# moble/scri

Measured on NVIDIA B200. Metric: mode-timesteps/sec through WaveformModes.transform (ell_max=8), higher is better.
Workload: dtype f64

## Files before the change

### scri_b200/csrc/spline_tile.cu

```cuda
#include <cuda.h>
#include <math_constants.h>
#include <stdlib.h>

#include "common.cuh"

namespace scrib200 {

constexpr int ST_COLS = 16;
constexpr int ST_ROWD = 16;
constexpr int ST_BR = 16;
constexpr int ST_TAB6 = 6;
constexpr int FACTOR_RUNIN = 40;
constexpr int ST_MAXBLK = 24;

__device__ __forceinline__ unsigned st_smem_u32(const void* p) { return (unsigned)__cvta_generic_to_shared(p); }

__device__ __forceinline__ int st_idx(int rrel, int c) { return rrel * ST_ROWD + ((((c >> 1) ^ (rrel & 7)) << 1) | (c & 1)); }

__device__ __forceinline__ void nak_row(const double* __restrict__ t, int N, int r, double& sub, double& diag, double& sup,
                                        double& hm, double& hp) {
    hm = t[r] - t[r - 1];
    hp = t[r + 1] - t[r];
    sub = hm;
    diag = 2.0 * (hm + hp);
// ... 245 lines not shown
        int total = 0;
#pragma unroll
        for (int c = 0; c < ST_COLS / 2; ++c) total += s_nch[c];
        const int per = (total + nwarp - 1) / nwarp;
        el = warp * per;
        erem = (total - el < per) ? total - el : per;
        while (ec < ST_COLS / 2 && el >= s_nch[ec]) el -= s_nch[ec++];
        if (erem > 0 && ec < ST_COLS / 2) {
            const int jn = s_jlo[ec] + (el << 5) + lane;
            if (jn < s_jhi[ec]) u_next = up[jn];
        }
    }
    {
        unsigned ok = 0;
        const unsigned mb = st_smem_u32(&s_mbar);
        while (!ok)
            asm volatile("{ .reg .pred p; mbarrier.try_wait.parity.shared::cta.b64 p, [%1], 0; selp.u32 %0, 1, 0, p; }" : "=r"(ok) : "r"(mb) : "memory");
    }

    const int cc = tid & (ST_COLS - 1);
    const int q = qlo + tid / ST_COLS;
    const bool active = (q <= qhi);
    const int qbase = q * ST_BR;
    const int r0 = (qbase > slo) ? qbase : slo;
    const int r1 = (qbase + ST_BR - 1 < shi) ? qbase + ST_BR - 1 : shi;
    const bool full = active && r0 == qbase && r1 == qbase + ST_BR - 1;
    const int rb = qbase - ybase;
    const int c2 = cc >> 1, c1 = cc & 1;
    const double* yq = sY + rb * ST_ROWD + c1;
    double* mq = sD + rb * ST_ROWD + c1;
    const double* tq = sTab + rb * ST_TAB6;
#define YQ(k_) yq[(k_) * ST_ROWD + ((c2 ^ ((k_) & 7)) << 1)]
#define MQ(k_) mq[(k_) * ST_ROWD + ((c2 ^ ((k_) & 7)) << 1)]
#define TQ2(k_, f_) (*reinterpret_cast<const double2*>(tq + (k_) * ST_TAB6 + (f_)))
    double dreg[ST_BR];
    if (full) {
        double yc = YQ(0);
        double dym = yc - YQ(-1);
        double d = 0.0;
#pragma unroll
        for (int k = 0; k < ST_BR; ++k) {
            const double yn = YQ(k + 1);
            const double dy = yn - yc;
            const double2 pq = TQ2(k, 0);
            d = fma(-tq[k * ST_TAB6 + 4], d, pq.x * dy - pq.y * dym);
            dreg[k] = d;
            yc = yn;
            dym = dy;
        }
        sEdgeD[(q - qlo) * ST_COLS + cc] = d;
    } else if (active) {
        double yc = SY(r0, cc);
        double dym = yc - SY(r0 - 1, cc);
        double d = 0.0;
#pragma unroll
        for (int k = 0; k < ST_BR; ++k) {
            dreg[k] = 0.0;
            if (qbase + k >= r0 && qbase + k <= r1) {
                const double yn = YQ(k + 1);
                const double dy = yn - yc;
                const double2 pq = TQ2(k, 0);
                d = fma(-tq[k * ST_TAB6 + 4], d, pq.x * dy - pq.y * dym);
                dreg[k] = d;
                yc = yn;
                dym = dy;
            }
        }
        sEdgeD[(q - qlo) * ST_COLS + cc] = d;
    }
    __syncthreads();
    if (active) {
        double D = 0.0, w = 1.0;
        for (int p = q - 1; p >= qlo; --p) {
            D = fma(w, sEdgeD[(p - qlo) * ST_COLS + cc], D);
            w *= STAB(p * ST_BR + ST_BR - 1, 2);
            if (fabs(w) < 1e-24) break;
        }
        double m = 0.0;
        if (full) {
#pragma unroll
            for (int k = ST_BR - 1; k >= 0; --k) {
                const double2 pc = TQ2(k, 2);
                m = fma(-pc.y, m, fma(pc.x, D, dreg[k]));
                dreg[k] = m;
            }
        } else {
#pragma unroll
            for (int k = ST_BR - 1; k >= 0; --k)
                if (qbase + k >= r0 && qbase + k <= r1) {
                    const double2 pc = TQ2(k, 2);
                    m = fma(-pc.y, m, fma(pc.x, D, dreg[k]));
                    dreg[k] = m;
                }
        }
        sEdgeM[(q - qlo) * ST_COLS + cc] = m;
    }
    __syncthreads();
    if (active) {
        double E = 0.0, w = 1.0;
        for (int p = q + 1; p <= qhi; ++p) {
            E = fma(w, sEdgeM[(p - qlo) * ST_COLS + cc], E);
            w *= STAB(p * ST_BR, 5);
            if (fabs(w) < 1e-24) break;
        }
        if (full) {
#pragma unroll
            for (int k = 0; k < ST_BR; ++k) MQ(k) = fma(tq[k * ST_TAB6 + 5], E, dreg[k]);
        } else {
#pragma unroll
            for (int k = 0; k < ST_BR; ++k)
                if (qbase + k >= r0 && qbase + k <= r1) MQ(k) = fma(tq[k * ST_TAB6 + 5], E, dreg[k]);
        }
    }
#undef YQ
#undef MQ
#undef TQ2
    __syncthreads();
    if (a == 0 && tid < ST_COLS) {
        const double h0 = STT(1) - STT(0), h1 = STT(2) - STT(1);
        SD(0, tid) = ((h0 + h1) * SD(1, tid) - h0 * SD(2, tid)) / h1;
    }
    if (last_tile && tid >= 32 && tid < 32 + ST_COLS) {
        const int c = tid - 32;
        const double hm = STT(N - 2) - STT(N - 3), hp = STT(N - 1) - STT(N - 2);
        SD(N - 1, c) = ((hm + hp) * SD(N - 2, c) - hp * SD(N - 3, c)) / hm;
    }
    if (a == 0 || last_tile) __syncthreads();

    if (MODE == 0) {
        double2* o2 = reinterpret_cast<double2*>(out);
        const int tmask = (1 << tshift) - 1;
        const int64_t jbase = (int64_t)bz * Nout;
        const int64_t ostride = ((int64_t)32 >> tshift) * ((int64_t)G << tshift);
        while (erem > 0 && ec < ST_COLS / 2) {
            const int c = ec;
            const int nrun = (s_nch[c] - el < erem) ? s_nch[c] - el : erem;
            const int j1 = s_jhi[c];
            const int g = bx * (ST_COLS / 2) + c;
            const double k = s_k[c], al = s_al[c], xa = s_xa[c];
            const float slope = s_slope[c];
            int j = s_jlo[c] + (el << 5) + lane;
            const int64_t jg0 = jbase + j;
            double2* optr = o2 + ((((jg0 >> tshift) * G + g) << tshift) + (jg0 & tmask));
            double u = u_next;
            for (int run = 0; run < nrun; ++run, j += 32, optr += ostride) {
                if (run + 1 < nrun) {
                    u_next = (j + 32 < j1) ? up[j + 32] : 0.0;
                }
                if (j < j1) {
            int i = a + __float2int_rd((float)(u - xa) * slope);
            i = max(a, min(i, b - 1));
            double ti = STT(i), ti1 = STT(i + 1);
            double xi = __dmul_rn(k, __dsub_rn(ti, al));
            double xi1 = __dmul_rn(k, __dsub_rn(ti1, al));
            if (!((xi <= u || i == a) && (u < xi1 || i == b - 1))) {
                int lo_s = a, hi_s = b - 1;
                while (lo_s < hi_s) {
                    const int mid = (lo_s + hi_s + 1) >> 1;
                    if (__dmul_rn(k, __dsub_rn(STT(mid), al)) <= u) lo_s = mid; else hi_s = mid - 1;
                }
                i = lo_s;
                ti = STT(i);
                ti1 = STT(i + 1);
                xi = __dmul_rn(k, __dsub_rn(ti, al));
                xi1 = __dmul_rn(k, __dsub_rn(ti1, al));
            }
            const double ht = ti1 - ti;
            const double hx = xi1 - xi;
            float seed;
            asm("rcp.approx.ftz.f32 %0, %1;" : "=f"(seed) : "f"((float)hx));
            double inv_h = (double)seed;
            double e = fma(-hx, inv_h, 1.0);
            if (fabs(e) < 1e-3) {
                inv_h = fma(inv_h, e, inv_h);
                e = fma(-hx, inv_h, 1.0);
                inv_h = fma(inv_h, e, inv_h);
            } else {
                inv_h = 1.0 / hx;
            }
            const double A = (xi1 - u) * inv_h;
            const double B = (u - xi) * inv_h;
            const double h26 = ht * ht * (1.0 / 6.0);
            const double ca = (A * A * A - A) * h26;
            const double cb = (B * B * B - B) * h26;
            const int ir = i - ybase;
            const int o0 = ir * ST_ROWD + ((c ^ (ir & 7)) << 1), o1 = (ir + 1) * ST_ROWD + ((c ^ ((ir + 1) & 7)) << 1);
            const double2 yi = *reinterpret_cast<const double2*>(sY + o0);
            const double2 yi1 = *reinterpret_cast<const double2*>(sY + o1);
            const double2 Mi = *reinterpret_cast<const double2*>(sD + o0);
            const double2 Mi1 = *reinterpret_cast<const double2*>(sD + o1);
            double2 r;
            r.x = A * yi.x + B * yi1.x + (ca * Mi.x + cb * Mi1.x);
            r.y = A * yi.y + B * yi1.y + (ca * Mi.y + cb * Mi1.y);
                    *optr = r;
                }
                u = u_next;
            }
            erem -= nrun;
            el = 0;
            ++ec;
            if (erem > 0 && ec < ST_COLS / 2) {
                const int jn = s_jlo[ec] + lane;
                u_next = (jn < s_jhi[ec]) ? up[jn] : 0.0;
            }
        }
    } else {
        const int rstep = nthr / ST_COLS;
        const bool colok = col0 + cc < G2;
        out += (size_t)bz * N * G2;
        if (MODE == 4) up += (size_t)bz * N * G2;
        auto value = [&](int i, bool& last_row, double& last_val) -> double {
            const double ht = STT(i + 1) - STT(i);
            const double yi = SY(i, cc), yi1 = SY(i + 1, cc);
            const double Mi = SD(i, cc), Mi1 = SD(i + 1, cc);
            last_row = false;
            if (MODE == 1) {
                const double dl = (yi1 - yi) / ht, h6 = ht * (1.0 / 6.0);
                if (i == N - 2) {
                    last_row = true;
                    last_val = dl + h6 * (Mi + 2.0 * Mi1);
                }
                return dl - h6 * (2.0 * Mi + Mi1);
            } else if (MODE == 2) {
                if (i == N - 2) {
                    last_row = true;
                    last_val = Mi1;
                }
                return Mi;
            } else if (MODE == 3) {
                return 0.5 * ht * (yi + yi1) - (ht * ht * ht) * (1.0 / 24.0) * (Mi + Mi1);
            } else {
                const double c1 = (yi1 - yi) / ht - ht * (1.0 / 6.0) * (2.0 * Mi + Mi1);
                const double h2 = ht * ht;
                const double Jv = h2 * (0.5 * yi + ht * (1.0 / 6.0) * c1 + h2 * ((1.0 / 24.0) * Mi + (1.0 / 120.0) * (Mi1 - Mi)));
                return Jv + (colok ? ht * up[(size_t)i * G2 + col0 + cc] : 0.0);
            }
        };
        if (MODE <= 2) {
            for (int i = a + tid / ST_COLS; i < b; i += rstep) {
                bool lr;
                double lv = 0.0;
                const double v = value(i, lr, lv);
                if (!colok) continue;
                out[(size_t)i * G2 + col0 + cc] = v;
                if (lr) out[(size_t)(N - 1) * G2 + col0 + cc] = lv;
            }
        } else {
            constexpr int VMAX = 16;
            double val[VMAX];
            bool lr;
            double lv;
#pragma unroll
            for (int k = 0; k < VMAX; ++k) {
                const int i = a + tid / ST_COLS + k * rstep;
                val[k] = (i < b) ? value(i, lr, lv) : 0.0;
            }
            __syncthreads();
#pragma unroll
            for (int k = 0; k < VMAX; ++k) {
                const int i = a + tid / ST_COLS + k * rstep;
                if (i < b) SD(i, cc) = val[k];
            }
            __syncthreads();
            const int nr = b - a, slen = (nr + ST_BR - 1) / ST_BR;
            for (int id = tid; id < ST_BR * ST_COLS; id += nthr) {
                const int s = id / ST_COLS, c = id - s * ST_COLS;
                const int r0s = a + s * slen, r1s = (r0s + slen < b) ? r0s + slen : b;
                double run = 0.0;
                for (int r = r0s; r < r1s; ++r) {
                    run += SD(r, c);
                    SD(r, c) = run;
                }
                sEdgeD[s * ST_COLS + c] = run;
            }
            __syncthreads();
            if (tid < ST_COLS) {
                double run = 0.0;
#pragma unroll
                for (int p = 0; p < ST_BR; ++p) {
                    const double v = sEdgeD[p * ST_COLS + tid];
                    sEdgeD[p * ST_COLS + tid] = run;
                    run += v;
                }
            }
            __syncthreads();
            if (colok) {
                const float rs = 1.0f / (float)slen;
                for (int i = a + tid / ST_COLS; i < b; i += rstep) {
                    int s = (int)((float)(i - a) * rs);
                    s -= (s * slen > i - a);
                    s += ((s + 1) * slen <= i - a);
                    out[(size_t)(i + 1) * G2 + col0 + cc] = SD(i, cc) + sEdgeD[s * ST_COLS + cc];
                    if (i == 0) out[col0 + cc] = 0.0;
                }
            }
        }
    }
#undef SY
#undef SD
#undef STAB
#undef STT
}

__global__ void __launch_bounds__(1024)
tile_scan_totals_kernel(double* __restrict__ x, int64_t N, int C, int body, int ntiles) {
    __shared__ double tot[32][33];
    const int col = blockIdx.x * 32 + threadIdx.x, seg = threadIdx.y;
    const int per = (ntiles + 31) / 32;
    const int k0 = seg * per, k1 = (k0 + per < ntiles) ? k0 + per : ntiles;
    const bool ok = col < C;
    auto at = [&](int k) -> double* {
        const int64_t last = (int64_t)(k + 1) * body;
        return x + (last < N - 1 ? last : N - 1) * C + col;
    };
    double run = 0.0;
    if (ok) {
        for (int k = k0; k < k1; k += 8) {
            double v[8];
#pragma unroll
            for (int j = 0; j < 8; ++j) v[j] = (k + j < k1) ? *at(k + j) : 0.0;
#pragma unroll
            for (int j = 0; j < 8; ++j)
                if (k + j < k1) {
                    run += v[j];
                    *at(k + j) = run;
                }
        }
    }
    tot[seg][threadIdx.x] = run;
    __syncthreads();
    if (!ok || seg == 0) return;
    double pre = 0.0;
    for (int p = 0; p < seg; ++p) pre += tot[p][threadIdx.x];
    for (int k = k0; k < k1; k += 8) {
        double v[8];
#pragma unroll
        for (int j = 0; j < 8; ++j) v[j] = (k + j < k1) ? *at(k + j) : 0.0;
#pragma unroll
        for (int j = 0; j < 8; ++j)
            if (k + j < k1) *at(k + j) = v[j] + pre;
    }
}

__global__ void __launch_bounds__(128)
tile_scan_add_kernel(double* __restrict__ x, int64_t N, int C, int body) {
    const int col = blockIdx.x * 128 + threadIdx.x;
    if (col >= C) return;
    const int64_t first = (int64_t)(blockIdx.y + 1) * body;
    if (first >= N - 1) return;
    const int64_t last = first + body < N - 1 ? first + body : N - 1;
    const double base = x[first * C + col];
    double* p = x + (first + 1) * C + col;
    int left = (int)(last - first - 1);
    for (; left >= 8; left -= 8, p += 8 * (size_t)C) {
        double v[8];
#pragma unroll
        for (int j = 0; j < 8; ++j) v[j] = p[(size_t)j * C];
#pragma unroll
        for (int j = 0; j < 8; ++j) p[(size_t)j * C] = v[j] + base;
    }
    for (; left > 0; --left, p += C) *p += base;
}

static int launch_tile_scan(double* x, int64_t N, int C, int body, cudaStream_t st) {
    const unsigned gx = (unsigned)((C + 127) / 128);
    const int64_t ntiles = (N - 1 + body - 1) / body;
    if (ntiles <= 1) return SCRIB200_OK;
    tile_scan_totals_kernel<<<(unsigned)((C + 31) / 32), dim3(32, 32), 0, st>>>(x, N, C, body, (int)ntiles);
    SCRIB200_CHECK_LAUNCH("spline_calculus(scan: totals)");
    tile_scan_add_kernel<<<dim3(gx, (unsigned)(ntiles - 1)), 128, 0, st>>>(x, N, C, body);
    SCRIB200_CHECK_LAUNCH("spline_calculus(scan: add)");
    return SCRIB200_OK;
}

static int tile_box_rows(int body, int halo) {
    const int ymax = body + 2 * halo + 2;
    return (((ymax + 7 + 1) / 2) + 7) & ~7;
}

static size_t tile_smem_bytes(int body, int halo) {
    const size_t nrows = 2 * (size_t)tile_box_rows(body, halo);
    const size_t nblk = std::max<size_t>(((size_t)body + 2 * halo) / ST_BR, ST_BR);
    return (2 * nrows * ST_ROWD + nrows * ST_TAB6 + nrows + 2 * nblk * ST_COLS + 5 * ST_COLS) * sizeof(double) + 1024;
}

static void resolve_tile(int& halo, int& body) {
    if (halo <= 0) halo = 32;
    if (body <= 0) {
        static const int env_body = [] { const char* e = std::getenv("SCRIB200_TILE_BODY"); return e ? std::atoi(e) : 0; }();
        body = env_body > 0 ? env_body : ((halo <= 32) ? 240 : (halo <= 64 ? 176 : 128));
    }
}

typedef CUresult (*TensorMapEncodeTiledFn)(CUtensorMap*, CUtensorMapDataType, cuuint32_t, void*, const cuuint64_t*, const cuuint64_t*,
                                            const cuuint32_t*, const cuuint32_t*, CUtensorMapInterleave, CUtensorMapSwizzle,
                                            CUtensorMapL2promotion, CUtensorMapFloatOOBfill);

static TensorMapEncodeTiledFn tensor_map_encoder() {
    static TensorMapEncodeTiledFn fn = nullptr;
    if (fn == nullptr) {
        void* p = nullptr;
        cudaDriverEntryPointQueryResult qres;
        if (cudaGetDriverEntryPoint("cuTensorMapEncodeTiled", &p, cudaEnableDefault, &qres) == cudaSuccess && qres == cudaDriverEntryPointSuccess)
            fn = reinterpret_cast<TensorMapEncodeTiledFn>(p);
    }
    return fn;
}

template <int MODE>
static int launch_tile(const double* t, int64_t n_times, const double* F, int G, const double* kconf, const double* alpha,
                       const double* tab, const double* uprm, int64_t n_out, double* out, int tshift, int halo, int body,
                       void* workspace, size_t workspace_bytes, void* stream, const char* name, int n_series = 1,
                       int64_t row_lo = 0, int64_t row_hi = -1) {
    SCRIB200_REQUIRE(n_times < (int64_t)2147483000 && n_out < (int64_t)2147483000, "%s: series longer than 2^31 samples", name);
    resolve_tile(halo, body);
    SCRIB200_REQUIRE(halo % ST_BR == 0 && body % ST_BR == 0, "%s: body=%d and halo=%d must be multiples of %d", name, body, halo, ST_BR);
    const size_t smem = tile_smem_bytes(body, halo);
    const int nblk = (body + 2 * halo) / ST_BR;
    const int box_rows = tile_box_rows(body, halo);
    SCRIB200_REQUIRE(nblk <= ST_MAXBLK && smem <= 220 * 1024 && box_rows <= 256, "%s: body=%d halo=%d does not fit one CTA", name, body, halo);
    const int64_t ntiles = (n_times - 1 + body - 1) / body;
    SCRIB200_REQUIRE(ntiles <= 65535, "%s: too many time tiles (%lld); raise `body`", name, (long long)ntiles);
    SCRIB200_REQUIRE(n_series >= 1 && n_series <= 65535 && (int64_t)n_series * n_times < (int64_t)2147483000,
                     "%s: n_series=%d (x %lld rows) out of range", name, n_series, (long long)n_times);
    TensorMapEncodeTiledFn encode = tensor_map_encoder();
    SCRIB200_REQUIRE(encode != nullptr, "%s: cuTensorMapEncodeTiled is not available from this driver", name);
    CUtensorMap tmF;
    {
        const cuuint64_t gdim[2] = {(cuuint64_t)(2 * (int64_t)G), (cuuint64_t)((int64_t)n_series * n_times)};
        const cuuint64_t gstride[1] = {(cuuint64_t)(2 * (int64_t)G) * sizeof(double)};
        const cuuint32_t box[2] = {(cuuint32_t)ST_COLS, (cuuint32_t)box_rows};
        const cuuint32_t estr[2] = {1, 1};
        const CUresult r = encode(&tmF, CU_TENSOR_MAP_DATA_TYPE_FLOAT64, 2, const_cast<double*>(F), gdim, gstride, box, estr,
                                  CU_TENSOR_MAP_INTERLEAVE_NONE, CU_TENSOR_MAP_SWIZZLE_128B, CU_TENSOR_MAP_L2_PROMOTION_L2_128B,
                                  CU_TENSOR_MAP_FLOAT_OOB_FILL_NONE);
        SCRIB200_REQUIRE(r == CUDA_SUCCESS, "%s: cuTensorMapEncodeTiled failed (%d) for a [%lld, %d] grid array", name, (int)r,
                         (long long)n_series * n_times, 2 * G);
    }
    const int threads = ((nblk * ST_COLS + 31) / 32) * 32;
    const bool small = threads <= 320;
    if (small) cudaFuncSetAttribute(spline_tile_kernel<MODE, 320>, cudaFuncAttributeMaxDynamicSharedMemorySize, (int)smem);
    else cudaFuncSetAttribute(spline_tile_kernel<MODE, ST_MAXBLK * ST_COLS>, cudaFuncAttributeMaxDynamicSharedMemorySize, (int)smem);
    int64_t tile_lo = 0, tile_hi = ntiles;
    if (row_hi >= 0) {
        tile_lo = (row_lo > 0 ? row_lo : 0) / body;
        tile_hi = (row_hi + body - 1) / body;
        if (tile_hi > ntiles) tile_hi = ntiles;
        if (tile_lo >= tile_hi) return SCRIB200_OK;
    }
    dim3 grid((2 * G + ST_COLS - 1) / ST_COLS, (unsigned)(tile_hi - tile_lo), (unsigned)n_series);
    int* J = nullptr;
    int* flags = nullptr;
    if (MODE == 0) {
        const size_t need = ((size_t)(ntiles + 1) * G + (size_t)ntiles * grid.x) * sizeof(int);
        SCRIB200_REQUIRE(workspace && workspace_bytes >= need, "%s: workspace too small (%zu < %zu)", name, workspace_bytes, need);
        J = reinterpret_cast<int*>(workspace);
        const int64_t total = (ntiles + 1) * (int64_t)G;
        spline_jrange_kernel<<<(unsigned)((total + 255) / 256), 256, 0, (cudaStream_t)stream>>>(
            t, (int)n_times, G, kconf, alpha, uprm, (int)n_out, body, (int)ntiles, J);
        SCRIB200_CHECK_LAUNCH(name);
        flags = J + total;
        const int64_t nflags = ntiles * (int64_t)grid.x;
        spline_tile_flags_kernel<<<(unsigned)((nflags + 255) / 256), 256, 0, (cudaStream_t)stream>>>(J, (int)ntiles, G, (int)grid.x, flags);
        SCRIB200_CHECK_LAUNCH(name);
    }
    if (small)
        spline_tile_kernel<MODE, 320><<<grid, threads, smem, (cudaStream_t)stream>>>(
            tmF, t, (int)n_times, G, kconf, alpha, tab, uprm, (int)n_out, out, tshift, body, halo, J, flags, box_rows, (int)tile_lo);
    else
        spline_tile_kernel<MODE, ST_MAXBLK * ST_COLS><<<grid, threads, smem, (cudaStream_t)stream>>>(
            tmF, t, (int)n_times, G, kconf, alpha, tab, uprm, (int)n_out, out, tshift, body, halo, J, flags, box_rows, (int)tile_lo);
    SCRIB200_CHECK_LAUNCH(name);
    return SCRIB200_OK;
}

}

extern "C" int scrib200_spline_prepare(const double* t, int64_t n_times, double gamma_factor, int divide, double time_translation,
                                       const double* kconf, const double* alpha, int G, double* tab, double* uprm,
                                       double* info, void* stream) {
    using namespace scrib200;
    SCRIB200_REQUIRE(t && tab && info, "spline_prepare: null pointer");
    SCRIB200_REQUIRE(n_times >= 4 && n_times < (int64_t)2147483000, "spline_prepare: a cubic interpolating spline needs at least 4 knots; got %lld",
                     (long long)n_times);
    SCRIB200_REQUIRE(uprm == nullptr || (kconf && alpha && G > 0), "spline_prepare: output times need kconf, alpha, G");
    SCRIB200_REQUIRE(aligned16(tab), "spline_prepare: tab must be 16-byte aligned");
    cudaStream_t st = (cudaStream_t)stream;
    spline_info_init_kernel<<<1, 32, 0, st>>>(info, (double)n_times);
    const unsigned blocks = (unsigned)((n_times + 255) / 256);
    spline_factor_kernel<<<blocks, 256, 0, st>>>(t, (int)n_times, tab, gamma_factor, divide,
                                                 time_translation, kconf, alpha, G, uprm, info);
    SCRIB200_CHECK_LAUNCH("spline_prepare(factor)");
    spline_decay_kernel<<<blocks, 256, 0, st>>>(tab, (int)n_times, info);
    SCRIB200_CHECK_LAUNCH("spline_prepare(decay)");
    return SCRIB200_OK;
}

extern "C" size_t scrib200_spline_remap_workspace_bytes(int64_t n_times, int G, int halo, int body) {
    using namespace scrib200;
    resolve_tile(halo, body);
    if (n_times < 2 || body <= 0) return 16;
    const int64_t ntiles = (n_times - 1 + body - 1) / body;
    const size_t ncg = (size_t)(2 * G + ST_COLS - 1) / ST_COLS;
    return ((size_t)(ntiles + 1) * (size_t)G + (size_t)ntiles * ncg) * sizeof(int) + 16;
}

extern "C" int scrib200_spline_remap(const double* t, int64_t n_times, const double* F, int G, const double* kconf,
                                     const double* alpha, const double* tab, const double* uprm, int64_t n_out,
                                     double* out, int tile, int halo, int body, int n_series, void* workspace,
                                     size_t workspace_bytes, void* stream) {
    using namespace scrib200;
    SCRIB200_REQUIRE(t && F && kconf && alpha && tab && uprm && out, "spline_remap: null pointer");
    SCRIB200_REQUIRE(n_times >= 4, "spline_remap: a cubic interpolating spline needs at least 4 knots; got %lld",
                     (long long)n_times);
    int tshift = 0;
    while ((1 << tshift) < tile) ++tshift;
    SCRIB200_REQUIRE(G > 0 && (tile == 0 || (tile >= 2 && tile <= 32 && (1 << tshift) == tile)),
                     "spline_remap: G=%d, tile=%d must be 0 (time-major output) or a power of two in 2..32", G, tile);
    SCRIB200_REQUIRE(aligned16(F) && aligned16(out) && aligned16(tab), "spline_remap: pointers must be 16-byte aligned");
    if (n_out <= 0) return SCRIB200_OK;
    return launch_tile<0>(t, n_times, F, G, kconf, alpha, tab, uprm, n_out, out, tile ? tshift : 0, halo, body, workspace,
                          workspace_bytes, stream, "spline_remap", n_series);
}

extern "C" int scrib200_spline_remap_rows(const double* t, int64_t n_times, const double* F, int G, const double* kconf,
                                          const double* alpha, const double* tab, const double* uprm, int64_t n_out,
                                          double* out, int tile, int halo, int body, int n_series, int64_t row_lo,
                                          int64_t row_hi, void* workspace, size_t workspace_bytes, void* stream) {
    using namespace scrib200;
    SCRIB200_REQUIRE(t && F && kconf && alpha && tab && uprm && out, "spline_remap_rows: null pointer");
    SCRIB200_REQUIRE(n_times >= 4, "spline_remap_rows: a cubic interpolating spline needs at least 4 knots; got %lld", (long long)n_times);
    int tshift = 0;
    while ((1 << tshift) < tile) ++tshift;
    SCRIB200_REQUIRE(G > 0 && (tile == 0 || (tile >= 2 && tile <= 32 && (1 << tshift) == tile)),
                     "spline_remap_rows: G=%d, tile=%d must be 0 (time-major output) or a power of two in 2..32", G, tile);
    SCRIB200_REQUIRE(aligned16(F) && aligned16(out) && aligned16(tab), "spline_remap_rows: pointers must be 16-byte aligned");
    SCRIB200_REQUIRE(row_lo >= 0 && row_hi >= row_lo, "spline_remap_rows: rows [%lld, %lld)", (long long)row_lo, (long long)row_hi);
    if (n_out <= 0) return SCRIB200_OK;
    return launch_tile<0>(t, n_times, F, G, kconf, alpha, tab, uprm, n_out, out, tile ? tshift : 0, halo, body, workspace,
                          workspace_bytes, stream, "spline_remap_rows", n_series, row_lo, row_hi);
}

extern "C" int scrib200_spline_calculus(const double* t, int64_t n_times, const double* data, int ncol,
                                        const double* tab, int order, double* out, double* aux, int halo, int body,
                                        void* stream) {
    using namespace scrib200;
    SCRIB200_REQUIRE(t && data && tab && out, "spline_calculus: null pointer");
    SCRIB200_REQUIRE(n_times >= 4, "spline_calculus: a cubic spline needs at least 4 knots; got %lld", (long long)n_times);
    SCRIB200_REQUIRE(order == 1 || order == 2 || order == -1 || order == -2,
                     "spline_calculus: order must be 1, 2 (derivatives) or -1, -2 (antiderivatives)");
    SCRIB200_REQUIRE(order != -2 || aux, "spline_calculus: order -2 needs `aux` [n_times, ncol] (receives the first antiderivative)");
    SCRIB200_REQUIRE(ncol > 0, "spline_calculus: ncol=%d", ncol);
    SCRIB200_REQUIRE(aligned16(data) && aligned16(out) && aligned16(tab) && aligned16(aux), "spline_calculus: pointers must be 16-byte aligned");
    if (order == 1)
        return launch_tile<1>(t, n_times, data, ncol, nullptr, nullptr, tab, nullptr, 0, out, 0, halo, body, nullptr, 0, stream, "spline_calculus");
    if (order == 2)
        return launch_tile<2>(t, n_times, data, ncol, nullptr, nullptr, tab, nullptr, 0, out, 0, halo, body, nullptr, 0, stream, "spline_calculus");
    const int C = 2 * ncol;
    double* first = (order == -1) ? out : aux;
    int rbody = body, rhalo = halo;
    resolve_tile(rhalo, rbody);
    int rc = launch_tile<3>(t, n_times, data, ncol, nullptr, nullptr, tab, nullptr, 0, first, 0, halo, body, nullptr, 0, stream, "spline_calculus");
    if (rc != SCRIB200_OK) return rc;
    rc = launch_tile_scan(first, n_times, C, rbody, (cudaStream_t)stream);
    if (rc != SCRIB200_OK) return rc;
    if (order == -1) return SCRIB200_OK;
    rc = launch_tile<4>(t, n_times, data, ncol, nullptr, nullptr, tab, first, 0, out, 0, halo, body, nullptr, 0, stream, "spline_calculus");
    if (rc != SCRIB200_OK) return rc;
    return launch_tile_scan(out, n_times, C, rbody, (cudaStream_t)stream);
}
```

Before: 3.307 billion.

## Add persistent warp-specialized pipelined spline remap kernel with mbarrier stages

Adds a persistent spline remap kernel used by default for MODE 0. Within each CTA, a producer warp issues TMA loads into multi-stage shared buffers, sweep warps solve the tridiagonal second-derivative system, and evaluator warps interpolate outputs. The stages are coordinated with mbarriers so loading, solving and evaluation of consecutive tiles overlap. It launches one CTA per SM with large shared memory and keeps the legacy kernel reachable through environment variables. A dev A/B script is also added.

Result: no change. 3.281 billion, median of 6 (-0.8%).

```diff
diff --git a/dev/dev_spline_ab.py b/dev/dev_spline_ab.py
--- /dev/null
+++ b/dev/dev_spline_ab.py
@@ -0,0 +1,78 @@
+import json, os, sys
+sys.path.insert(0, os.path.dirname(os.path.dirname(os.path.abspath(__file__))))
+sys.path.insert(0, os.path.join(os.path.dirname(os.path.dirname(os.path.abspath(__file__))), "tests"))
+import numpy as np, torch
+import scri_b200 as sb
+from scri_b200 import ops, plan as P
+from scri_inputs import real_supertranslation, smooth_modes
+
+rounds = int(sys.argv[1]) if len(sys.argv) > 1 else 60
+N = 100000
+t = np.linspace(0, 1e4, N)
+_, data = smooth_modes(n_times=N, t0=0.0, t1=1e4)
+kw = dict(supertranslation=real_supertranslation(4), frame_rotation=[1.0, 2.0, 3.0, 4.0], boost_velocity=[0.01, 0.02, 0.03])
+pl = P.TransformPlan(2, 8, sb.h, **kw)
+td = ops.to_device(t); ad = ops.to_device(data)
+prep = pl.prepare(td); F = pl.synthesize(ad); up = prep.uprm
+n_out = up.shape[0]
+print("n_out", n_out, "G", pl.G, "tile", pl.tile, "halo/body", prep.halo_body())
+flush = torch.empty(256 * 1024 * 1024, dtype=torch.uint8, device="cuda")
+VARIANTS = {"legacy": {"SCRIB200_SPLINE_LEGACY": "1"}, "pipe3x1_e8": {"SCRIB200_SPLINE_PIPE": "0"},
+            "pipe2x2_e8": {"SCRIB200_SPLINE_PIPE": "1"}, "pipe3x1_e6": {"SCRIB200_SPLINE_PIPE": "2"}}
+
+
+def use(name):
+    for k in ("SCRIB200_SPLINE_LEGACY", "SCRIB200_SPLINE_PIPE"):
+        os.environ.pop(k, None)
+    os.environ.update(VARIANTS[name])
+
+
+def rows(g):
+    return g.permute(0, 2, 1).reshape(-1, pl.G)[:n_out]
+
+
+outs = {}
+for name in VARIANTS:
+    use(name)
+    for _ in range(3):
+        g = pl.remap_tiled(td, F, up, prep)
+    torch.cuda.synchronize()
+    outs[name] = rows(g).clone()
+equal = {name: bool(torch.equal(outs[name], outs["legacy"])) for name in VARIANTS}
+print("bit-identical to legacy:", equal)
+
+times = {name: [] for name in VARIANTS}
+for r in range(rounds):
+    for name in VARIANTS:
+        use(name)
+        flush.fill_(r & 255)
+        e0, e1 = torch.cuda.Event(enable_timing=True), torch.cuda.Event(enable_timing=True)
+        torch.cuda._sleep(int(2e7))
+        e0.record(); pl.remap_tiled(td, F, up, prep); e1.record()
+        torch.cuda.synchronize()
+        times[name].append(e0.elapsed_time(e1))
+
+kernel_ms = {}
+for name in VARIANTS:
+    use(name)
+    with torch.profiler.profile(activities=[torch.profiler.ProfilerActivity.CUDA]) as prof:
+        for r in range(10):
+            flush.fill_(r)
+            pl.remap_tiled(td, F, up, prep)
+        torch.cuda.synchronize()
+    per = {}
+    for e in prof.key_averages():
+        if "spline" in e.key and e.count:
+            per[e.key.split("(")[0][:80]] = (getattr(e, "device_time_total", None) or e.cuda_time_total) / e.count / 1e3
+    kernel_ms[name] = per
+
+res = {"n_out": int(n_out), "G": pl.G, "rounds": rounds, "bit_identical_to_legacy": equal, "call_ms": {}, "kernel_ms": kernel_ms}
+for name, ts in times.items():
+    a = np.array(ts)
+    res["call_ms"][name] = {"median": float(np.median(a)), "min": float(a.min()), "max": float(a.max()),
+                            "p10": float(np.percentile(a, 10)), "p90": float(np.percentile(a, 90))}
+    print(f"{name:12s} spline_remap call: median {np.median(a):.4f} ms  [min {a.min():.4f}, p10 {np.percentile(a, 10):.4f}, "
+          f"p90 {np.percentile(a, 90):.4f}, max {a.max():.4f}]  kernels: " + ", ".join(f"{k} {v:.4f}" for k, v in kernel_ms[name].items()))
+if len(sys.argv) > 2:
+    with open(sys.argv[2], "w") as f:
+        json.dump(res, f, indent=1)
diff --git a/scri_b200/csrc/spline_tile.cu b/scri_b200/csrc/spline_tile.cu
--- a/scri_b200/csrc/spline_tile.cu
+++ b/scri_b200/csrc/spline_tile.cu
@@ -571,6 +571,396 @@
 #undef STT
 }
 
+constexpr int SP_SWEEP = 320;
+constexpr int SP_SWEEP_WARPS = SP_SWEEP / 32;
+constexpr int SP_MAXBLK = SP_SWEEP / ST_COLS;
+
+struct SpConst {
+    double k[ST_COLS / 2], al[ST_COLS / 2], xa[ST_COLS / 2];
+    float slope[ST_COLS / 2];
+    int jlo[ST_COLS / 2], jhi[ST_COLS / 2], nch[ST_COLS / 2];
+};
+
+__device__ __forceinline__ void sp_mb_wait(unsigned mb, unsigned parity) {
+    unsigned ok = 0;
+    while (!ok)
+        asm volatile("{ .reg .pred p; mbarrier.try_wait.parity.shared::cta.b64 p, [%1], %2; selp.u32 %0, 1, 0, p; }"
+                     : "=r"(ok) : "r"(mb), "r"(parity) : "memory");
+}
+__device__ __forceinline__ void sp_mb_arrive(unsigned mb) {
+    asm volatile("mbarrier.arrive.shared::cta.b64 _, [%0];" ::"r"(mb) : "memory");
+}
+
+__device__ __forceinline__ bool sp_item(int64_t w, int ncg, int ntl, int tile_off, const int* __restrict__ flags, int& bx,
+                                        int& by, int& bz) {
+    const int64_t r = w / ncg;
+    bx = (int)(w - r * ncg);
+    const int64_t s = r / ntl;
+    by = (int)(r - s * ntl) + tile_off;
+    bz = (int)s;
+    return flags[(size_t)by * ncg + bx] != 0;
+}
+
+template <int NF, int NM, int NE>
+__global__ void __launch_bounds__(SP_SWEEP + 32 * NE + 32, 1)
+spline_remap_pipe_kernel(const __grid_constant__ CUtensorMap tmF, const double* __restrict__ t, int N, int G,
+                         const double* __restrict__ kconf, const double* __restrict__ alpha,
+                         const double* __restrict__ tab, const double* __restrict__ up, int Nout,
+                         double* __restrict__ out, int tshift, int body, int halo, const int* __restrict__ J,
+                         const int* __restrict__ flags, int box_rows, int tile_off, int ntl, int n_series) {
+    extern __shared__ unsigned char s_raw[];
+    const int tid = threadIdx.x, lane = tid & 31, warp = tid >> 5;
+    const int ncg = (2 * G + ST_COLS - 1) / ST_COLS;
+    const int64_t nitems = (int64_t)n_series * ntl * ncg;
+    const int nrows = 2 * box_rows;
+
+    double* const sY0 = reinterpret_cast<double*>(s_raw + ((1024u - (st_smem_u32(s_raw) & 1023u)) & 1023u));
+    double* const sD0 = sY0 + (size_t)NF * nrows * ST_ROWD;
+    double* const sTab0 = sD0 + (size_t)NM * nrows * ST_ROWD;
+    double* const sT0 = sTab0 + (size_t)NF * nrows * ST_TAB6;
+    double* const sEdgeD = sT0 + (size_t)NF * nrows;
+    double* const sEdgeM = sEdgeD + SP_MAXBLK * ST_COLS;
+    SpConst* const sC0 = reinterpret_cast<SpConst*>(sEdgeM + SP_MAXBLK * ST_COLS);
+    unsigned long long* const mbar = reinterpret_cast<unsigned long long*>(sC0 + NF);
+    const unsigned fullF = st_smem_u32(mbar), emptyF = fullF + 8 * NF, fullM = emptyF + 8 * NF, emptyM = fullM + 8 * NM;
+
+    if (tid == 0) {
+        for (int s = 0; s < NF; ++s) {
+            asm volatile("mbarrier.init.shared::cta.b64 [%0], %1;" ::"r"(fullF + 8 * s), "r"(32));
+            asm volatile("mbarrier.init.shared::cta.b64 [%0], %1;" ::"r"(emptyF + 8 * s), "r"(SP_SWEEP_WARPS + NE));
+        }
+        for (int m = 0; m < NM; ++m) {
+            asm volatile("mbarrier.init.shared::cta.b64 [%0], %1;" ::"r"(fullM + 8 * m), "r"(SP_SWEEP_WARPS));
+            asm volatile("mbarrier.init.shared::cta.b64 [%0], %1;" ::"r"(emptyM + 8 * m), "r"(NE));
+        }
+        asm volatile("fence.mbarrier_init.release.cluster;" ::: "memory");
+    }
+    __syncthreads();
+
+    if (warp == SP_SWEEP_WARPS + NE) {
+        int n = 0;
+        for (int64_t w = blockIdx.x; w < nitems; w += gridDim.x) {
+            int bx, by, bz;
+            if (!sp_item(w, ncg, ntl, tile_off, flags, bx, by, bz)) continue;
+            const int s = n % NF;
+            if (n >= NF) sp_mb_wait(emptyF + 8 * s, (unsigned)((n / NF - 1) & 1));
+            const int a = by * body;
+            const int b = (a + body < N - 1) ? a + body : N - 1;
+            const int slo = (a - halo > 1) ? a - halo : 1;
+            const int shi = (b + halo - 1 < N - 2) ? b + halo - 1 : N - 2;
+            const int ylo = slo - 1, yhi = shi + 1;
+            const int ybase = ylo & ~7;
+            double* const sY = sY0 + (size_t)s * nrows * ST_ROWD;
+            double* const sT = sT0 + (size_t)s * nrows;
+            if (lane == 0) {
+                const unsigned mb = fullF + 8 * s;
+                const int trows = ((yhi < N - 1) ? yhi : N - 1) - ybase + 1;
+                const unsigned tab_bytes = (unsigned)trows * ST_TAB6 * (unsigned)sizeof(double);
+                const unsigned box_bytes = (unsigned)box_rows * ST_ROWD * (unsigned)sizeof(double);
+                asm volatile("mbarrier.expect_tx.shared::cta.b64 [%0], %1;" ::"r"(mb), "r"(2u * box_bytes + tab_bytes) : "memory");
+                const int row0 = bz * N + ybase;
+#pragma unroll
+                for (int h2 = 0; h2 < 2; ++h2)
+                    asm volatile(
+                        "cp.async.bulk.tensor.2d.shared::cluster.global.mbarrier::complete_tx::bytes [%0], [%1, {%2, %3}], [%4];" ::"r"(
+                            st_smem_u32(sY) + h2 * box_bytes),
+                        "l"(&tmF), "r"(bx * ST_COLS), "r"(row0 + h2 * box_rows), "r"(mb)
+                        : "memory");
+                asm volatile("cp.async.bulk.shared::cluster.global.mbarrier::complete_tx::bytes [%0], [%1], %2, [%3];" ::"r"(
+                                 st_smem_u32(sTab0 + (size_t)s * nrows * ST_TAB6)),
+                             "l"(tab + (size_t)ybase * ST_TAB6), "r"(tab_bytes), "r"(mb)
+                             : "memory");
+            }
+            for (int e = lane; e <= yhi - ybase; e += 32) sT[e] = t[ybase + e];
+            if (lane < ST_COLS / 2) {
+                SpConst& C = sC0[s];
+                const int c = lane;
+                const int g = bx * (ST_COLS / 2) + c;
+                const bool ok = g < G;
+                const double k = ok ? kconf[g] : 1.0, al = ok ? alpha[g] : 0.0;
+                C.k[c] = k;
+                C.al[c] = al;
+                int jlo = 0, jhi = 0;
+                if (ok) {
+                    const double xa = __dmul_rn(k, __dsub_rn(t[a], al));
+                    const double xbv = __dmul_rn(k, __dsub_rn(t[b], al));
+                    C.xa[c] = xa;
+                    C.slope[c] = (float)((double)(b - a) / (xbv - xa));
+                    jlo = J[(size_t)by * G + g];
+                    jhi = J[(size_t)(by + 1) * G + g];
+                }
+                C.jlo[c] = jlo;
+                C.jhi[c] = jhi;
+                C.nch[c] = (jhi - jlo + 31) >> 5;
+            }
+            sp_mb_arrive(fullF + 8 * s);
+            ++n;
+        }
+        return;
+    }
+
+    if (warp < SP_SWEEP_WARPS) {
+        const int cc = tid & (ST_COLS - 1);
+        const int c2 = cc >> 1, c1 = cc & 1;
+        int n = 0;
+        for (int64_t w = blockIdx.x; w < nitems; w += gridDim.x) {
+            int bx, by, bz;
+            if (!sp_item(w, ncg, ntl, tile_off, flags, bx, by, bz)) continue;
+            const int s = n % NF, m = n % NM;
+            const int a = by * body;
+            const int b = (a + body < N - 1) ? a + body : N - 1;
+            const bool last_tile = (b == N - 1);
+            const int slo = (a - halo > 1) ? a - halo : 1;
+            const int shi = (b + halo - 1 < N - 2) ? b + halo - 1 : N - 2;
+            const int ybase = (slo - 1) & ~7;
+            const int qlo = slo / ST_BR, qhi = shi / ST_BR;
+            const double* const sY = sY0 + (size_t)s * nrows * ST_ROWD;
+            double* const sD = sD0 + (size_t)m * nrows * ST_ROWD;
+            const double* const sTab = sTab0 + (size_t)s * nrows * ST_TAB6;
+            const double* const sT = sT0 + (size_t)s * nrows;
+#define SY(r_, c_) sY[st_idx((r_) - ybase, (c_))]
+#define SD(r_, c_) sD[st_idx((r_) - ybase, (c_))]
+#define STAB(r_, f_) sTab[((r_) - ybase) * ST_TAB6 + (f_)]
+#define STT(r_) sT[(r_) - ybase]
+            const int q = qlo + tid / ST_COLS;
+            const bool active = (q <= qhi);
+            const int qbase = q * ST_BR;
+            const int r0 = (qbase > slo) ? qbase : slo;
+            const int r1 = (qbase + ST_BR - 1 < shi) ? qbase + ST_BR - 1 : shi;
+            const bool full = active && r0 == qbase && r1 == qbase + ST_BR - 1;
+            const int rb = qbase - ybase;
+            const double* yq = sY + rb * ST_ROWD + c1;
+            double* mq = sD + rb * ST_ROWD + c1;
+            const double* tq = sTab + rb * ST_TAB6;
+#define YQ(k_) yq[(k_) * ST_ROWD + ((c2 ^ ((k_) & 7)) << 1)]
+#define MQ(k_) mq[(k_) * ST_ROWD + ((c2 ^ ((k_) & 7)) << 1)]
+#define TQ2(k_, f_) (*reinterpret_cast<const double2*>(tq + (k_) * ST_TAB6 + (f_)))
+            sp_mb_wait(fullF + 8 * s, (unsigned)((n / NF) & 1));
+            double dreg[ST_BR];
+            if (full) {
+                double yc = YQ(0);
+                double dym = yc - YQ(-1);
+                double d = 0.0;
+#pragma unroll
+                for (int k = 0; k < ST_BR; ++k) {
+                    const double yn = YQ(k + 1);
+                    const double dy = yn - yc;
+                    const double2 pq = TQ2(k, 0);
+                    d = fma(-tq[k * ST_TAB6 + 4], d, pq.x * dy - pq.y * dym);
+                    dreg[k] = d;
+                    yc = yn;
+                    dym = dy;
+                }
+                sEdgeD[(q - qlo) * ST_COLS + cc] = d;
+            } else if (active) {
+                double yc = SY(r0, cc);
+                double dym = yc - SY(r0 - 1, cc);
+                double d = 0.0;
+#pragma unroll
+                for (int k = 0; k < ST_BR; ++k) {
+                    dreg[k] = 0.0;
+                    if (qbase + k >= r0 && qbase + k <= r1) {
+                        const double yn = YQ(k + 1);
+                        const double dy = yn - yc;
+                        const double2 pq = TQ2(k, 0);
+                        d = fma(-tq[k * ST_TAB6 + 4], d, pq.x * dy - pq.y * dym);
+                        dreg[k] = d;
+                        yc = yn;
+                        dym = dy;
+                    }
+                }
+                sEdgeD[(q - qlo) * ST_COLS + cc] = d;
+            }
+            asm volatile("bar.sync 1, %0;" ::"n"(SP_SWEEP) : "memory");
+            if (active) {
+                double D = 0.0, wgt = 1.0;
+                for (int p = q - 1; p >= qlo; --p) {
+                    D = fma(wgt, sEdgeD[(p - qlo) * ST_COLS + cc], D);
+                    wgt *= STAB(p * ST_BR + ST_BR - 1, 2);
+                    if (fabs(wgt) < 1e-24) break;
+                }
+                double mm = 0.0;
+                if (full) {
+#pragma unroll
+                    for (int k = ST_BR - 1; k >= 0; --k) {
+                        const double2 pc = TQ2(k, 2);
+                        mm = fma(-pc.y, mm, fma(pc.x, D, dreg[k]));
+                        dreg[k] = mm;
+                    }
+                } else {
+#pragma unroll
+                    for (int k = ST_BR - 1; k >= 0; --k)
+                        if (qbase + k >= r0 && qbase + k <= r1) {
+                            const double2 pc = TQ2(k, 2);
+                            mm = fma(-pc.y, mm, fma(pc.x, D, dreg[k]));
+                            dreg[k] = mm;
+                        }
+                }
+                sEdgeM[(q - qlo) * ST_COLS + cc] = mm;
+            }
+            asm volatile("bar.sync 1, %0;" ::"n"(SP_SWEEP) : "memory");
+            if (active) {
+                double E = 0.0, wgt = 1.0;
+                for (int p = q + 1; p <= qhi; ++p) {
+                    E = fma(wgt, sEdgeM[(p - qlo) * ST_COLS + cc], E);
+                    wgt *= STAB(p * ST_BR, 5);
+                    if (fabs(wgt) < 1e-24) break;
+                }
+                if (n >= NM) sp_mb_wait(emptyM + 8 * m, (unsigned)((n / NM - 1) & 1));
+                if (full) {
+#pragma unroll
+                    for (int k = 0; k < ST_BR; ++k) MQ(k) = fma(tq[k * ST_TAB6 + 5], E, dreg[k]);
+                } else {
+#pragma unroll
+                    for (int k = 0; k < ST_BR; ++k)
+                        if (qbase + k >= r0 && qbase + k <= r1) MQ(k) = fma(tq[k * ST_TAB6 + 5], E, dreg[k]);
+                }
+            }
+#undef YQ
+#undef MQ
+#undef TQ2
+            if (a == 0 || last_tile) {
+                asm volatile("bar.sync 1, %0;" ::"n"(SP_SWEEP) : "memory");
+                if (a == 0 && tid < ST_COLS) {
+                    const double h0 = STT(1) - STT(0), h1 = STT(2) - STT(1);
+                    SD(0, tid) = ((h0 + h1) * SD(1, tid) - h0 * SD(2, tid)) / h1;
+                }
+                if (last_tile && tid >= 32 && tid < 32 + ST_COLS) {
+                    const int c = tid - 32;
+                    const double hm = STT(N - 2) - STT(N - 3), hp = STT(N - 1) - STT(N - 2);
+                    SD(N - 1, c) = ((hm + hp) * SD(N - 2, c) - hp * SD(N - 3, c)) / hm;
+                }
+            }
+#undef SY
+#undef SD
+#undef STAB
+#undef STT
+            __syncwarp();
+            if (lane == 0) {
+                sp_mb_arrive(fullM + 8 * m);
+                sp_mb_arrive(emptyF + 8 * s);
+            }
+            ++n;
+        }
+        return;
+    }
+
+    const int ew = warp - SP_SWEEP_WARPS;
+    double2* const o2 = reinterpret_cast<double2*>(out);
+    const int tmask = (1 << tshift) - 1;
+    const int64_t ostride = ((int64_t)32 >> tshift) * ((int64_t)G << tshift);
+    int n = 0;
+    for (int64_t w = blockIdx.x; w < nitems; w += gridDim.x) {
+        int bx, by, bz;
+        if (!sp_item(w, ncg, ntl, tile_off, flags, bx, by, bz)) continue;
+        const int s = n % NF, m = n % NM;
+        const int a = by * body;
+        const int b = (a + body < N - 1) ? a + body : N - 1;
+        const int slo = (a - halo > 1) ? a - halo : 1;
+        const int ybase = (slo - 1) & ~7;
+        const double* const sY = sY0 + (size_t)s * nrows * ST_ROWD;
+        const double* const sD = sD0 + (size_t)m * nrows * ST_ROWD;
+        const double* const sT = sT0 + (size_t)s * nrows;
+        const SpConst& C = sC0[s];
+#define STT(r_) sT[(r_) - ybase]
+        sp_mb_wait(fullF + 8 * s, (unsigned)((n / NF) & 1));
+        int ec = 0, el = 0, erem = 0;
+        double u_next = 0.0;
+        {
+            int total = 0;
+#pragma unroll
+            for (int c = 0; c < ST_COLS / 2; ++c) total += C.nch[c];
+            const int per = (total + NE - 1) / NE;
+            el = ew * per;
+            erem = (total - el < per) ? total - el : per;
+            while (ec < ST_COLS / 2 && el >= C.nch[ec]) el -= C.nch[ec++];
+            if (erem > 0 && ec < ST_COLS / 2) {
+                const int jn = C.jlo[ec] + (el << 5) + lane;
+                if (jn < C.jhi[ec]) u_next = up[jn];
+            }
+        }
+        sp_mb_wait(fullM + 8 * m, (unsigned)((n / NM) & 1));
+        const int64_t jbase = (int64_t)bz * Nout;
+        while (erem > 0 && ec < ST_COLS / 2) {
+            const int c = ec;
+            const int nrun = (C.nch[c] - el < erem) ? C.nch[c] - el : erem;
+            const int j1 = C.jhi[c];
+            const int g = bx * (ST_COLS / 2) + c;
+            const double k = C.k[c], al = C.al[c], xa = C.xa[c];
+            const float slope = C.slope[c];
+            int j = C.jlo[c] + (el << 5) + lane;
+            const int64_t jg0 = jbase + j;
+            double2* optr = o2 + ((((jg0 >> tshift) * G + g) << tshift) + (jg0 & tmask));
+            double u = u_next;
+            for (int run = 0; run < nrun; ++run, j += 32, optr += ostride) {
+                if (run + 1 < nrun) u_next = (j + 32 < j1) ? up[j + 32] : 0.0;
+                if (j < j1) {
+                    int i = a + __float2int_rd((float)(u - xa) * slope);
+                    i = max(a, min(i, b - 1));
+                    double ti = STT(i), ti1 = STT(i + 1);
+                    double xi = __dmul_rn(k, __dsub_rn(ti, al));
+                    double xi1 = __dmul_rn(k, __dsub_rn(ti1, al));
+                    if (!((xi <= u || i == a) && (u < xi1 || i == b - 1))) {
+                        int lo_s = a, hi_s = b - 1;
+                        while (lo_s < hi_s) {
+                            const int mid = (lo_s + hi_s + 1) >> 1;
+                            if (__dmul_rn(k, __dsub_rn(STT(mid), al)) <= u) lo_s = mid; else hi_s = mid - 1;
+                        }
+                        i = lo_s;
+                        ti = STT(i);
+                        ti1 = STT(i + 1);
+                        xi = __dmul_rn(k, __dsub_rn(ti, al));
+                        xi1 = __dmul_rn(k, __dsub_rn(ti1, al));
+                    }
+                    const double ht = ti1 - ti;
+                    const double hx = xi1 - xi;
+                    float seed;
+                    asm("rcp.approx.ftz.f32 %0, %1;" : "=f"(seed) : "f"((float)hx));
+                    double inv_h = (double)seed;
+                    double e = fma(-hx, inv_h, 1.0);
+                    if (fabs(e) < 1e-3) {
+                        inv_h = fma(inv_h, e, inv_h);
+                        e = fma(-hx, inv_h, 1.0);
+                        inv_h = fma(inv_h, e, inv_h);
+                    } else {
+                        inv_h = 1.0 / hx;
+                    }
+                    const double A = (xi1 - u) * inv_h;
+                    const double B = (u - xi) * inv_h;
+                    const double h26 = ht * ht * (1.0 / 6.0);
+                    const double ca = (A * A * A - A) * h26;
+                    const double cb = (B * B * B - B) * h26;
+                    const int ir = i - ybase;
+                    const int o0 = ir * ST_ROWD + ((c ^ (ir & 7)) << 1), o1 = (ir + 1) * ST_ROWD + ((c ^ ((ir + 1) & 7)) << 1);
+                    const double2 yi = *reinterpret_cast<const double2*>(sY + o0);
+                    const double2 yi1 = *reinterpret_cast<const double2*>(sY + o1);
+                    const double2 Mi = *reinterpret_cast<const double2*>(sD + o0);
+                    const double2 Mi1 = *reinterpret_cast<const double2*>(sD + o1);
+                    double2 r;
+                    r.x = A * yi.x + B * yi1.x + (ca * Mi.x + cb * Mi1.x);
+                    r.y = A * yi.y + B * yi1.y + (ca * Mi.y + cb * Mi1.y);
+                    *optr = r;
+                }
+                u = u_next;
+            }
+            erem -= nrun;
+            el = 0;
+            ++ec;
+            if (erem > 0 && ec < ST_COLS / 2) {
+                const int jn = C.jlo[ec] + lane;
+                u_next = (jn < C.jhi[ec]) ? up[jn] : 0.0;
+            }
+        }
+#undef STT
+        __syncwarp();
+        if (lane == 0) {
+            sp_mb_arrive(emptyM + 8 * m);
+            sp_mb_arrive(emptyF + 8 * s);
+        }
+        ++n;
+    }
+}
+
 __global__ void __launch_bounds__(1024)
 tile_scan_totals_kernel(double* __restrict__ x, int64_t N, int C, int body, int ntiles) {
     __shared__ double tot[32][33];
@@ -674,6 +1064,36 @@
             fn = reinterpret_cast<TensorMapEncodeTiledFn>(p);
     }
     return fn;
+}
+
+static size_t pipe_smem_bytes(int box_rows, int NF, int NM) {
+    const size_t nrows = 2 * (size_t)box_rows;
+    return (NF * nrows * (ST_ROWD + ST_TAB6 + 1) + NM * nrows * ST_ROWD + 2 * SP_MAXBLK * ST_COLS) * sizeof(double) +
+           NF * sizeof(SpConst) + (2 * NF + 2 * NM) * sizeof(unsigned long long) + 1024;
+}
+
+template <int NF, int NM, int NE>
+static int launch_pipe(const CUtensorMap& tmF, const double* t, int64_t n_times, int G, const double* kconf, const double* alpha,
+                       const double* tab, const double* uprm, int64_t n_out, double* out, int tshift, int body, int halo,
+                       const int* J, const int* flags, int box_rows, int64_t tile_lo, int64_t tile_hi, int n_series, void* stream,
+                       const char* name) {
+    const size_t smem = pipe_smem_bytes(box_rows, NF, NM);
+    if (smem > 227 * 1024) return -1;
+    static int n_sm = 0;
+    if (n_sm == 0) {
+        int dev = 0;
+        cudaGetDevice(&dev);
+        cudaDeviceGetAttribute(&n_sm, cudaDevAttrMultiProcessorCount, dev);
+    }
+    const int ncg = (2 * G + ST_COLS - 1) / ST_COLS;
+    const int64_t nitems = (int64_t)n_series * (tile_hi - tile_lo) * ncg;
+    const unsigned blocks = (unsigned)(nitems < n_sm ? nitems : n_sm);
+    cudaFuncSetAttribute(spline_remap_pipe_kernel<NF, NM, NE>, cudaFuncAttributeMaxDynamicSharedMemorySize, (int)smem);
+    spline_remap_pipe_kernel<NF, NM, NE><<<blocks, SP_SWEEP + 32 * NE + 32, smem, (cudaStream_t)stream>>>(
+        tmF, t, (int)n_times, G, kconf, alpha, tab, uprm, (int)n_out, out, tshift, body, halo, J, flags, box_rows, (int)tile_lo,
+        (int)(tile_hi - tile_lo), n_series);
+    SCRIB200_CHECK_LAUNCH(name);
+    return SCRIB200_OK;
 }
 
 template <int MODE>
@@ -733,6 +1153,21 @@
         spline_tile_flags_kernel<<<(unsigned)((nflags + 255) / 256), 256, 0, (cudaStream_t)stream>>>(J, (int)ntiles, G, (int)grid.x, flags);
         SCRIB200_CHECK_LAUNCH(name);
     }
+    if (MODE == 0 && getenv("SCRIB200_SPLINE_LEGACY") == nullptr && nblk <= SP_MAXBLK) {
+        const char* pv = getenv("SCRIB200_SPLINE_PIPE");
+        const int variant = pv ? atoi(pv) : 0;
+        int rc = -1;
+        if (variant == 1)
+            rc = launch_pipe<2, 2, 8>(tmF, t, n_times, G, kconf, alpha, tab, uprm, n_out, out, tshift, body, halo, J, flags, box_rows,
+                                      tile_lo, tile_hi, n_series, stream, name);
+        else if (variant == 2)
+            rc = launch_pipe<3, 1, 6>(tmF, t, n_times, G, kconf, alpha, tab, uprm, n_out, out, tshift, body, halo, J, flags, box_rows,
+                                      tile_lo, tile_hi, n_series, stream, name);
+        else
+            rc = launch_pipe<3, 1, 8>(tmF, t, n_times, G, kconf, alpha, tab, uprm, n_out, out, tshift, body, halo, J, flags, box_rows,
+                                      tile_lo, tile_hi, n_series, stream, name);
+        if (rc >= 0) return rc;
+    }
     if (small)
         spline_tile_kernel<MODE, 320><<<grid, threads, smem, (cudaStream_t)stream>>>(
             tmF, t, (int)n_times, G, kconf, alpha, tab, uprm, (int)n_out, out, tshift, body, halo, J, flags, box_rows, (int)tile_lo);
```
